# sony/DiffRoll

Hardware: AMD Instinct MI355X
Metric: piano-roll frames/sec (200-step sample) (higher is better)
Workload: dtype f32

## Files before the change

### diffroll_amd/build.py

```python
from __future__ import annotations

import os
import shutil
import subprocess
import sys

HERE = os.path.dirname(os.path.abspath(__file__))
CSRC = os.path.join(HERE, "csrc")
LIBDIR = os.path.join(HERE, "lib")
LIB = os.path.join(LIBDIR, "libdiffroll_amd.so")
SOURCES = ["gemm.hip", "stack.hip", "tail.hip", "update.hip", "threshold.hip", "rescale.hip", "project.hip", "momentum.hip", "frontend.hip", "pack.hip", "plan.hip", "abi.hip", "debug_abi.hip", "comm.hip"]
HEADERS = [os.path.join(CSRC, h) for h in ("kernels.h", "chain_tables.h", "device_common.h", "gemm_body.h", "persistent.h", "update_quad.h", "threshold_quad.h", "rescale_quad.h", "project_quad.h", "momentum_quad.h", "engine_state.h", "device_buffer.h", "captured_chain.h", "fused_mode.h", "launch_plan.h", "tenants.h")] + \
          [os.path.join(os.path.dirname(HERE), "include", h) for h in ("diffroll_amd.h", "diffroll_amd_debug.h")]
FLAGS = ["--offload-arch=gfx950", "-O3", "-std=c++17", "-fPIC", "-Wall", "-Wno-unused-function"]


def _hipcc() -> str:
    for cand in (os.environ.get("HIPCC"), shutil.which("hipcc"), "/opt/rocm/bin/hipcc"):
        if cand and os.path.exists(cand):
            return cand
    raise RuntimeError("hipcc not found (need ROCm with gfx950 support)")


def _stale(target: str, deps) -> bool:
    if not os.path.exists(target):
        return True
    t = os.path.getmtime(target)
    return any(os.path.getmtime(d) > t for d in deps)


VARIANTS = {
    "bounds": dict(flags=["-DDR_BOUNDS"], link=[]),
    "hook": dict(flags=["-DDR_FAULT_HOOK"], link=[]),
    "fault1": dict(flags=["-DDR_FAULT=1"], link=[]),
    "fault2": dict(flags=["-DDR_FAULT=2"], link=[]),
    "asan": dict(flags=["-O1", "-g", "-fsanitize=address,undefined", "-fno-gpu-sanitize", "-shared-libsan", "-fno-omit-frame-pointer"],
                 link=["-fsanitize=address,undefined", "-shared-libsan"]),
    "ubsan": dict(flags=["-O1", "-g", "-fsanitize=undefined", "-fno-sanitize-recover=undefined", "-fno-gpu-sanitize", "-fno-omit-frame-pointer"],
                  link=["-fsanitize=undefined", "-shared-libsan", "@RPATH:libclang_rt.ubsan_standalone-x86_64.so"]),
}


def variant_path(variant: str) -> str:
    return os.path.join(LIBDIR, f"libdiffroll_amd_{variant}.so")


def build(force: bool = False, verbose: bool = True, variant: str = "") -> str:
    hipcc = _hipcc()
    os.makedirs(LIBDIR, exist_ok=True)
    objdir = os.path.join(LIBDIR, "obj" + ("_" + variant if variant else ""))
    os.makedirs(objdir, exist_ok=True)
    extra = VARIANTS[variant] if variant else dict(flags=[], link=[])
    lib = variant_path(variant) if variant else LIB
    objs = []
    relink = force
    jobs = []
    wanted = {src.replace(".hip", ".o") for src in SOURCES}
    for name in os.listdir(objdir):
        if name not in wanted:
            os.remove(os.path.join(objdir, name))
            relink = True
    for src in SOURCES:
        s = os.path.join(CSRC, src)
        o = os.path.join(objdir, src.replace(".hip", ".o"))
        if force or _stale(o, [s] + HEADERS):
            jobs.append([hipcc] + FLAGS + extra["flags"] + ["-c", s, "-o", o])
        objs.append(o)
    if jobs:
        from concurrent.futures import ThreadPoolExecutor

        def run(cmd):
            if verbose:
                print(" ".join(cmd), flush=True)
            subprocess.check_call(cmd)
        with ThreadPoolExecutor(max_workers=min(len(jobs), os.cpu_count() or 4)) as ex:
            list(ex.map(run, jobs))
        relink = True
    if relink or _stale(lib, objs):
        link = []
        for f in extra["link"]:
            if f.startswith("@RPATH:"):
                rt = subprocess.check_output([hipcc, "-print-file-name=" + f[len("@RPATH:"):]], text=True).strip()
                link.append("-Wl,-rpath," + os.path.dirname(os.path.realpath(rt)))
            else:
                link.append(f)
        cmd = [hipcc, "--offload-arch=gfx950", "-shared", "-fPIC"] + link + objs + ["-ldl", "-o", lib]
        if verbose:
            print(" ".join(cmd), flush=True)
        subprocess.check_call(cmd)
    return lib


def asan_runtime() -> str:
    out = subprocess.check_output([_hipcc(), "-print-file-name=libclang_rt.asan-x86_64.so"], text=True).strip()
    return out


if __name__ == "__main__":
    var = ""
    for a in sys.argv[1:]:
        if a.startswith("--variant="):
            var = a.split("=", 1)[1]
    print(build(force="--force" in sys.argv, variant=var))
```

### diffroll_amd/csrc/gemm_body.h

```cpp
#pragma once
#include "device_common.h"

namespace dr {

DR_DEVINL void residual_quad(const float (&v)[4], const float4 bias, const float4 prev, float (&o)[4]) {
    float bb[4], pv[4];
    f4arr(bias, bb); f4arr(prev, pv);
#pragma unroll
    for (int e = 0; e < 4; ++e) o[e] = div_sqrt2(pv[e] + (v[e] + bb[e]));
}
DR_DEVINL void skip_quad(const float (&v)[4], const float4 bias, const float4 prev, const bool skip_init, float (&o)[4]) {
    float bb[4], pv[4];
    f4arr(bias, bb); f4arr(prev, pv);
#pragma unroll
    for (int e = 0; e < 4; ++e) o[e] = skip_init ? v[e] + bb[e] : (v[e] + bb[e]) + pv[e];
}
DR_DEVINL long cond_row(const GemmArgs& a, const int b) {
    int r = a.c_b0 + b;
    if (a.c_n > 0 && r >= a.c_n) r %= a.c_n;
    return r;
}
DR_DEVINL void gate_quad(const float (&v0)[4], const float (&v1)[4], const float4 bias0, const float4 bias1,
                         const float4 cond0, const float4 cond1, const bool has_c, float (&o)[4]) {
    float b0[4], b1[4], c0[4], c1[4];
    f4arr(bias0, b0); f4arr(bias1, b1);
    f4arr(cond0, c0); f4arr(cond1, c1);
#pragma unroll
    for (int e = 0; e < 4; ++e) {
        const float a0 = has_c ? b0[e] + c0[e] : b0[e];
        const float a1 = has_c ? b1[e] + c1[e] : b1[e];
        o[e] = gatef_(v0[e] + a0, v1[e] + a1);
    }
}
DR_DEVINL void hd_quad(const float (&h)[4], const float4 d, float (&o)[4]) {
    float dd[4];
    f4arr(d, dd);
#pragma unroll
    for (int e = 0; e < 4; ++e) o[e] = h[e] + dd[e];
}
template <int COH3, int COH4, int BF = 0>
DR_DEVINL void store_y2(const GemmArgs& a, const int b, const float (&o)[4], const float4 d, const int p0, const int t) {
    float o2[4];
    hd_quad(o, d, o2);
    if constexpr (BF) {
        store_bf16_quad<COH3>(a.Y2 + (long)b * a.y2_bs, o2, p0, t, a.T, a.wt_store);
    } else if (a.out_s3 & 2) {
        store_s3_quad<COH3>(a.Y2 + (long)b * a.y2_bs, o2, p0, t, a.T, a.y_rows >> 3, a.wt_store);
    } else {
        float* dst2 = a.Y2 + (long)b * a.y2_bs + (long)(p0 >> 2) * a.y_ps + (long)t * a.y_fs;
        store_f4<COH4>(dst2, make_float4(o2[0], o2[1], o2[2], o2[3]), a.wt_store);
    }
}

DR_DEVINL AF4 load_a4(const __amdgpu_buffer_rsrc_t wrsrc, const int wvo, const int slab, const int NS, const int code) {
    AF4 o;
#pragma unroll
    for (int g = 0; g < 4; ++g) {
        DR_CHECK(slab >= 0 && wvo + slab * 16384 + g * 4096 + 16 <= NS * 16384, code, slab, NS);
        o.v[g] = buffer_load_f4(wrsrc, wvo, slab * 16384 + g * 4096);
    }
    return o;
}

typedef __attribute__((address_space(3))) void* lds_ptr;

template <int BN, int AUX, class PlaneOf>
DR_DEVINL void dma_tile(float4* Rs, PlaneOf plane_of, const int T, const int t0, const int first, const int stride, const int lane, const int code) {
    constexpr int RWL = (BN + 63) / 64;
    for (int i = first; i < 32 * RWL; i += stride) {
        const int pl = i / RWL, seg = i - pl * RWL;
        const int f = seg * 64 + lane;
        const __amdgpu_buffer_rsrc_t rsrc = __builtin_amdgcn_make_buffer_rsrc((void*)plane_of(pl), 0, (unsigned)T * 16u, 0x00020000);
        if (BN % 64 == 0 || f < BN) {
            DR_CHECK_LDS(Rs + pl * BN + f, lds_off(Rs), lds_off(Rs) + 32u * BN * 16u, code);
            __builtin_amdgcn_raw_ptr_buffer_load_lds(rsrc, (lds_ptr)(Rs + pl * BN + seg * 64), 16, (t0 + f) * 16, 0, 0, AUX);
        }
    }
}

template <int KS, int PREC, int AUX, int RBN>
DR_DEVINL void producer(const GemmArgs& a, float4* Xs, float4* Rs, const int pw, const int lane, const int mt, const int b, const int t0,
                        const int halo, const int FW, const int c0, const int c1, const int code_x, const int code_r) {
    constexpr int XP = (PREC == 2 ? 4 : PREC ? 12 : 8) * KS;
    const int bx = a.x_bmod ? (b % a.x_bmod) : b;
    const float* Xg = a.X + (long)bx * a.x_bs;
    const int last_plane = a.x_planes - 1;
    const unsigned recs = ((unsigned)(a.T - 1) * (unsigned)a.x_fs + 4u) * 4u;
    const int wl = (FW + 63) >> 6;
    const int total = XP * wl;
    auto issue = [&](int chunk) {
        for (int i = pw; i < total; i += 4) {
            const int pl = i / wl, seg = i - pl * wl;
            const int f = seg * 64 + lane;
            const float* src;
            if constexpr (PREC == 2) {
                const int pc = min(chunk * (4 * KS) + pl, last_plane);
                src = Xg + (long)pc * a.x_ps;
            } else if constexpr (PREC) {
                const int sg = pl / 6, rem = pl - sg * 6, pce = rem >> 1, kq = rem & 1;
                const int pc = min(chunk * (4 * KS) + sg * 2 + kq, last_plane);
                src = Xg + (long)pce * a.x_piece + (long)pc * a.x_ps;
            } else {
                src = Xg + (long)min(chunk * XP + pl, last_plane) * a.x_ps;
            }
            const __amdgpu_buffer_rsrc_t rsrc = __builtin_amdgcn_make_buffer_rsrc((void*)src, 0, recs, 0x00020000);
            const int voff = (t0 - halo + f) * (int)a.x_fs * 4;
            float4* dst = Xs + (((chunk - c0) & 1) * XP + pl) * FW + seg * 64;
            if (f < FW) DR_CHECK_LDS(dst + lane, lds_off(Xs), lds_off(Xs) + 2u * XP * FW * 16u, code_x);
            if (f < FW) __builtin_amdgcn_raw_ptr_buffer_load_lds(rsrc, (lds_ptr)dst, 16, voff, 0, 0, AUX);
        }
    };
    if constexpr (RBN != 0) {
        auto plane_of = [&](int pl) -> const float* {
            const int row0 = mt * 128 + pl * 4;
            return (row0 < a.y_rows) ? a.Y + (long)b * a.y_bs + (long)(row0 >> 2) * a.y_ps
                                     : a.skip + (long)b * a.s_bs + (long)((row0 - a.y_rows) >> 2) * a.T * 4;
        };
        dma_tile<RBN, AUX>(Rs, plane_of, a.T, t0, pw, 4, lane, code_r);
    }
    issue(c0);
    for (int chunk = c0; chunk < c1; ++chunk) {
#if DR_FAULT != 1
        asm volatile("s_waitcnt vmcnt(0)" ::: "memory");
        __syncthreads();
#else
        __builtin_amdgcn_s_barrier();
#endif
        if (chunk + 1 < c1) issue(chunk + 1);
    }
}

template <int NI, int KS, int EPI, int PREC, int COH, int FOLDP = (NI == 1)>
DR_DEVINL void gemm_body(const GemmArgs& a, char* smem, const int mt, const int nt, const int ks) {
    constexpr int NW = (NI == 3 || NI == 5) ? NI : 2 * NI;
    constexpr int BN = 32 * NW;
    static_assert(NI == 1 || NI == 2 || ((NI == 3 || NI == 5) && EPI == EPI_GATE && PREC == 0 && KS == 1 && FOLDP == 1),
                  "block widths: 64, 128; 96, 160 (conv)");
    constexpr int XP = (PREC == 2 ? 4 : PREC ? 12 : 8) * KS;
    constexpr bool PAIRED = (EPI == EPI_GATE || EPI == EPI_POWER);
    int tid = threadIdx.x;
    if constexpr (COH) asm volatile("" : "+v"(tid));
    const int lane = tid & 63;
    const int wave = __builtin_amdgcn_readfirstlane(tid >> 6);
    const long long tick0 = a.dbg ? clock64() : 0;

    const int halo = ((a.taps - 1) >> 1) * a.dil;
    const int FW = BN + 2 * halo;
    float4* Xs = reinterpret_cast<float4*>(smem);
    float4* Rs = Xs + 2 * XP * FW;
#ifdef DR_BOUNDS
    const unsigned xs0 = lds_off(Xs), xs1 = xs0 + 2u * XP * FW * 16u, rs1 = xs1 + (EPI == EPI_RES_SKIP ? 32u * BN * 16u : 0u);
    if (tid == 0 && !COH) DR_CHECK(rs1 <= (unsigned)a.lds_bytes, 100, rs1, a.lds_bytes);
#endif

    const int tps = (a.T + BN - 1) / BN;
    const int b = nt / tps;
    const int t0 = (nt % tps) * BN;
    const int NS = a.kchunks * a.taps;
    const int cps = a.kchunks / KS / a.ksplit;
    const int c0 = ks * cps, c1 = c0 + cps;

    if (wave >= 4) {
        producer<KS, PREC, COH ? 16 : 0, EPI == EPI_RES_SKIP ? BN : 0>(a, Xs, Rs, wave - 4, lane, mt, b, t0, halo, FW, c0, c1, 101, 102);
        return;
    }

    const int r = lane & 31, hi = lane >> 5;

    f32x16 acc[NW];
#pragma unroll
    for (int ni = 0; ni < NW; ++ni)
#pragma unroll
        for (int e = 0; e < 16; ++e) acc[ni][e] = 0.f;
    f32x16 outer[NW];
#pragma unroll
    for (int ni = 0; ni < NW; ++ni)
#pragma unroll
        for (int e = 0; e < 16; ++e) outer[ni][e] = 0.f;
    const f32x16 zero16 = {0.f, 0.f, 0.f, 0.f, 0.f, 0.f, 0.f, 0.f, 0.f, 0.f, 0.f, 0.f, 0.f, 0.f, 0.f, 0.f};
    constexpr bool FOLD = FOLDP && EPI == EPI_GATE;
    auto fold = [&]() {
        if constexpr (FOLD) {
#pragma unroll
            for (int ni = 0; ni < NW; ++ni) outer[ni] = outer[ni] + acc[ni];
#pragma unroll
            for (int ni = 0; ni < NW; ++ni) asm volatile("" : "+v"(outer[ni]));
        }
    };

    float4 eop[NW][4];

    if constexpr (PREC == 2) {
        const __amdgpu_buffer_rsrc_t wrsrc = __builtin_amdgcn_make_buffer_rsrc(
            (void*)(a.Wp + (long)mt * NS * 2048), 0, (unsigned)NS * 8192u, 0x00020000);
        const int wvo = (hi * 128 + wave * 32 + r) * 16;
        auto load_ag = [&](int slab, int g) -> uint4 {
            DR_CHECK(slab >= 0 && wvo + slab * 8192 + g * 4096 + 16 <= NS * 8192, 113, slab, NS);
            return buffer_load_u4(wrsrc, wvo, slab * 8192 + g * 4096);
        };
        const int s0 = c0 * KS * a.taps;
        AF2 wA, wB;
        wA.v[0] = load_ag(s0, 0); wA.v[1] = load_ag(s0, 1);
        wB.v[0] = load_ag(min(s0 + 1, NS - 1), 0); wB.v[1] = load_ag(min(s0 + 1, NS - 1), 1);
        const int cen = (a.taps - 1) >> 1;
        const int per_chunk = a.taps * KS;
        const uint4* Xsb = reinterpret_cast<const uint4*>(Xs);
        struct BF1 { uint4 v[NW]; };
        BF1 b0, b1;
        auto xaddr = [&](int chunk, int q) -> const uint4* {
            const int j = q / KS, sub = q - j * KS;
            return Xsb + (((chunk - c0) & 1) * XP + sub * 4 + hi) * FW + halo + (j - cen) * a.dil + r;
        };
        auto rd1 = [&](const uint4* Xb, int g) -> BF1 {
            BF1 o;
#pragma unroll
            for (int ni = 0; ni < NW; ++ni) {
                DR_CHECK_LDS(Xb + g * 2 * FW + ni * 32, xs0, xs1, 114);
                o.v[ni] = Xb[g * 2 * FW + ni * 32];
            }
            return o;
        };
        auto mma1 = [&](auto FIRST, const uint4 af, const BF1& bf) {
            constexpr bool kFirst = FOLD && decltype(FIRST)::value;
#pragma unroll
            for (int ni = 0; ni < NW; ++ni) acc[ni] = mma_bf16(af, bf.v[ni], kFirst ? zero16 : acc[ni]);
        };
        auto step = [&](auto ROLE, auto FIRST, int slab, int chunk, int q) {
            constexpr bool kB = decltype(ROLE)::value;
            const uint4* Xb = xaddr(chunk, q);
            const int nx = min(slab + 2, NS - 1);
            b1 = rd1(Xb, 1);
            mma1(FIRST, kB ? wB.v[0] : wA.v[0], b0);
            if constexpr (kB) wB.v[0] = load_ag(nx, 0);
            else wA.v[0] = load_ag(nx, 0);
            b0 = rd1(xaddr(chunk, min(q + 1, per_chunk - 1)), 0);
            mma1(std::false_type{}, kB ? wB.v[1] : wA.v[1], b1);
            if constexpr (kB) wB.v[1] = load_ag(nx, 1);
            else wA.v[1] = load_ag(nx, 1);
            sgb<0x100, 1>();
            sgb_mix1<NW - 1, 0>(); sgb<0x8, 1>(); sgb<0x20, 1>();
            sgb<0x100, 1>();
            sgb_mix1<NW - 1, 0>(); sgb<0x8, 1>(); sgb<0x20, 1>();
        };
        using T_ = std::true_type;
        using F_ = std::false_type;
        for (int chunk = c0; chunk < c1; ++chunk) {
            auto at = [&](auto R, auto FIRST, int q) {
                const int j = q / KS, sub = q - j * KS;
                step(R, FIRST, (chunk * KS + sub) * a.taps + j, chunk, q);
            };
            __syncthreads();
            b0 = rd1(xaddr(chunk, 0), 0);
            fold();
            at(F_{}, T_{}, 0);
            int q = 1;
            for (; q + 2 <= per_chunk; q += 2) {
                at(T_{}, F_{}, q);
                at(F_{}, F_{}, q + 1);
            }
            if (q < per_chunk) at(T_{}, F_{}, q);
            else { const AF2 t = wA; wA = wB; wB = t; }
        }
    } else if constexpr (PREC == 1) {
        const __amdgpu_buffer_rsrc_t wrsrc = __builtin_amdgcn_make_buffer_rsrc(
            (void*)(a.Wp + (long)mt * NS * 6144), 0, (unsigned)NS * 24576u, 0x00020000);
        const int wvo = (hi * 128 + wave * 32 + r) * 16;
        auto load_a3 = [&](int slab) -> AF6 {
            AF6 o;
#pragma unroll
            for (int gp = 0; gp < 6; ++gp) {
                DR_CHECK(slab >= 0 && wvo + slab * 24576 + gp * 4096 + 16 <= NS * 24576, 103, slab, NS);
                o.v[gp] = buffer_load_u4(wrsrc, wvo, slab * 24576 + gp * 4096);
            }
            return o;
        };
        AF6 wA = load_a3(c0 * KS * a.taps), wB;
        const int cen = (a.taps - 1) >> 1;
        const int per_chunk = a.taps * KS;
        const uint4* Xs3 = reinterpret_cast<const uint4*>(Xs);
        struct BF3 { uint4 v[3][NW]; };
        BF3 b0, b1;
        auto xaddr = [&](int chunk, int q) -> const uint4* {
            const int j = q / KS, sub = q - j * KS;
            return Xs3 + (((chunk - c0) & 1) * XP + sub * 12 + hi) * FW + halo + (j - cen) * a.dil + r;
        };
        auto rd3 = [&](const uint4* Xb, int g) -> BF3 {
            BF3 o;
#pragma unroll
            for (int pz = 0; pz < 3; ++pz)
#pragma unroll
                for (int ni = 0; ni < NW; ++ni) {
                    DR_CHECK_LDS(Xb + (g * 6 + pz * 2) * FW + ni * 32, xs0, xs1, 104);
                    o.v[pz][ni] = Xb[(g * 6 + pz * 2) * FW + ni * 32];
                }
            return o;
        };
        auto mma6 = [&](auto FIRST, const uint4 a0, const uint4 a1, const uint4 a2, const BF3& bf) {
            constexpr bool kFirst = FOLD && decltype(FIRST)::value;
#pragma unroll
            for (int ni = 0; ni < NW; ++ni) acc[ni] = mma_bf16(a2, bf.v[0][ni], kFirst ? zero16 : acc[ni]);
#pragma unroll
            for (int ni = 0; ni < NW; ++ni) acc[ni] = mma_bf16(a0, bf.v[2][ni], acc[ni]);
#pragma unroll
            for (int ni = 0; ni < NW; ++ni) acc[ni] = mma_bf16(a1, bf.v[1][ni], acc[ni]);
// ... 361 lines not shown
#pragma unroll
    for (int ni = 0; ni < NW; ++ni)
#pragma unroll
        for (int e = 0; e < 16; ++e) acc[ni][e] = 0.f;

    AF4 aA = load_a(0), aB;
    BF bA = load_b(0), bB;
    auto step = [&](auto ROLE, int slab) {
        constexpr bool kB = decltype(ROLE)::value;
        const int nxt = min(slab + 1, NS - 1);
        if constexpr (kB) { aA = load_a(nxt); bA = load_b(nxt); }
        else { aB = load_a(nxt); bB = load_b(nxt); }
#pragma unroll
        for (int g = 0; g < 4; ++g) {
            const float4 af = kB ? aB.v[g] : aA.v[g];
#pragma unroll
            for (int ni = 0; ni < NW; ++ni) acc[ni] = __builtin_amdgcn_mfma_f32_32x32x2f32(af.x, (kB ? bB.v[g][ni] : bA.v[g][ni]).x, acc[ni], 0, 0, 0);
#pragma unroll
            for (int ni = 0; ni < NW; ++ni) acc[ni] = __builtin_amdgcn_mfma_f32_32x32x2f32(af.y, (kB ? bB.v[g][ni] : bA.v[g][ni]).y, acc[ni], 0, 0, 0);
#pragma unroll
            for (int ni = 0; ni < NW; ++ni) acc[ni] = __builtin_amdgcn_mfma_f32_32x32x2f32(af.z, (kB ? bB.v[g][ni] : bA.v[g][ni]).z, acc[ni], 0, 0, 0);
#pragma unroll
            for (int ni = 0; ni < NW; ++ni) acc[ni] = __builtin_amdgcn_mfma_f32_32x32x2f32(af.w, (kB ? bB.v[g][ni] : bA.v[g][ni]).w, acc[ni], 0, 0, 0);
        }
        constexpr int NLD = 4 + 4 * NW, PER = (16 * NW) / NLD;
        sgb_spread<NLD, PER>();
        sgb<0x8, 16 * NW - NLD * PER>();
    };
    const int rowb = mt * 128 + wave * 32 + 4 * hi;
    const bool res_rows = rowb < a.y_rows;
    float4 ebias[4], ed2[4], eop[RLDS ? 1 : NW][4];
    auto load_epilogue = [&]() {
#pragma unroll
        for (int q = 0; q < 4; ++q) {
            ebias[q] = *reinterpret_cast<const float4*>(a.bias + rowb + 8 * q);
            if constexpr (EPI == EPI_RES_SKIP)
                ed2[q] = *reinterpret_cast<const float4*>(a.d2 + (a.tsel ? (long)a.tsel[b] * a.d2_ts : 0) + min(rowb + 8 * q, a.y_rows - 4));
        }
        if constexpr (RLDS || EPI != EPI_RES_SKIP) return;
        const float* base = res_rows ? a.Y + (long)b * a.y_bs + (long)(rowb >> 2) * a.y_ps
                                     : a.skip + (long)b * a.s_bs + (long)((rowb - a.y_rows) >> 2) * a.T * 4;
        const long qs = res_rows ? 2 * a.y_ps : (long)2 * a.T * 4;
        const long fs = res_rows ? a.y_fs : 4;
#pragma unroll
        for (int ni = 0; ni < NW; ++ni) {
            const int tc = min(t0 + ni * 32 + r, a.T - 1);
#pragma unroll
            for (int q = 0; q < 4; ++q) eop[ni][q] = *reinterpret_cast<const float4*>(base + q * qs + tc * fs);
        }
    };
    int slab = 0;
    const int pre = max(NS - 2, 0) & ~1;
    for (; slab < pre; slab += 2) {
        step(std::false_type{}, slab);
        step(std::true_type{}, slab + 1);
        if (a.dbg && slab == 0 && blockIdx.x == 0 && threadIdx.x == 0) a.dbg[2] = clock64() - tick0;
    }
    if (a.dbg && blockIdx.x == 0 && threadIdx.x == 0) a.dbg[3] = clock64() - tick0;
    if constexpr (!RLDS) load_epilogue();
    __builtin_amdgcn_sched_barrier(0);
    for (; slab + 2 <= NS; slab += 2) {
        step(std::false_type{}, slab);
        step(std::true_type{}, slab + 1);
    }
    if (slab < NS) step(std::false_type{}, slab);
    const long long tick1 = a.dbg ? clock64() : 0;
    if constexpr (RLDS) load_epilogue();

#pragma unroll
    for (int ni = 0; ni < NW; ++ni) {
        const int t = t0 + ni * 32 + r;
        if (t >= a.T) continue;
#pragma unroll
        for (int q = 0; q < 4; ++q) {
            const int p0 = rowb + 8 * q;
            float v[4], o[4];
#pragma unroll
            for (int e = 0; e < 4; ++e) v[e] = acc[ni][4 * q + e];
            if constexpr (EPI != EPI_RES_SKIP) {
                if (p0 >= a.y_rows) continue;
                float bb[4];
                f4arr(ebias[q], bb);
#pragma unroll
                for (int e = 0; e < 4; ++e) {
                    o[e] = a.alpha * v[e] + bb[e];
                    if constexpr (EPI == EPI_RELU) o[e] = fmaxf(o[e], 0.f);
                }
                float* dst = a.Y + (long)b * a.y_bs + (long)(p0 >> 2) * a.y_ps + (long)t * a.y_fs;
                store_f4<COH>(dst, make_float4(o[0], o[1], o[2], o[3]), a.wt_store);
                continue;
            }
            float4* rs = nullptr;
            if constexpr (RLDS) rs = Rs + (wave * 8 + 2 * q + hi) * BN + foff + ni * 32 + r;
#ifdef DR_BOUNDS
            if constexpr (RLDS) DR_CHECK_LDS(rs, lds_off(Rs), lds_off(Rs) + 32u * BN * 16u, 121);
#endif
            float4 pv;
            if constexpr (RLDS) pv = *rs;
            else pv = eop[ni][q];
            if (res_rows) {
                float* dst = a.Y + (long)b * a.y_bs + (long)(p0 >> 2) * a.y_ps + (long)t * a.y_fs;
                residual_quad(v, ebias[q], pv, o);
                if constexpr (RLDS) *rs = make_float4(o[0], o[1], o[2], o[3]);
                else *reinterpret_cast<float4*>(dst) = make_float4(o[0], o[1], o[2], o[3]);
                if (a.Y2) store_y2<0, COH>(a, b, o, ed2[q], p0, t);
            } else {
                float* dst = a.skip + (long)b * a.s_bs + ((long)((p0 - a.y_rows) >> 2) * a.T + t) * 4;
                skip_quad(v, ebias[q], pv, a.skip_init, o);
                if constexpr (RLDS) *rs = make_float4(o[0], o[1], o[2], o[3]);
                else *reinterpret_cast<float4*>(dst) = make_float4(o[0], o[1], o[2], o[3]);
            }
        }
    }
    if (a.dbg && blockIdx.x == 0 && threadIdx.x == 0) {
        a.dbg[0] = tick1 - tick0;
        a.dbg[1] = clock64() - tick0;
    }
}

template <int NJ, int KS, int EPI>
DR_DEVINL void gemm16_body(const GemmArgs& a, char* smem, const int mt, const int nt) {
    static_assert(EPI == EPI_GATE || EPI == EPI_RES_SKIP, "16x16 variant: hot kernels only");
    constexpr int BN = 32 * NJ;
    constexpr int XP = 8 * KS;
    constexpr int RT = 2;
    constexpr int CT = 2 * NJ;

    const int tid = threadIdx.x;
    const int lane = tid & 63;
    const int wave = __builtin_amdgcn_readfirstlane(tid >> 6);
    const int halo = ((a.taps - 1) >> 1) * a.dil;
    const int FW = BN + 2 * halo;
    float4* Xs = reinterpret_cast<float4*>(smem);
    float4* Rs = Xs + 2 * XP * FW;
#ifdef DR_BOUNDS
    const unsigned xs0 = lds_off(Xs), xs1 = xs0 + 2u * XP * FW * 16u, rs1 = xs1 + (EPI == EPI_RES_SKIP ? 32u * BN * 16u : 0u);
    if (tid == 0) DR_CHECK(rs1 <= (unsigned)a.lds_bytes, 140, rs1, a.lds_bytes);
#endif

    const int tps = (a.T + BN - 1) / BN;
    const int b = nt / tps;
    const int t0 = (nt % tps) * BN;
    const int NS = a.kchunks * a.taps;
    const int nchunks = a.kchunks / KS;

    if (wave >= 4) {
        producer<KS, 0, 0, EPI == EPI_RES_SKIP ? BN : 0>(a, Xs, Rs, wave - 4, lane, mt, b, t0, halo, FW, 0, nchunks, 141, 142);
        return;
    }

    const int li = lane & 15, kq = lane >> 4;
    float4 acc[RT][CT];
#pragma unroll
    for (int rt = 0; rt < RT; ++rt)
#pragma unroll
        for (int ct = 0; ct < CT; ++ct) acc[rt][ct] = f4zero();

    const __amdgpu_buffer_rsrc_t wrsrc = __builtin_amdgcn_make_buffer_rsrc(
        (void*)(a.Wp + (long)mt * NS * 4096), 0, (unsigned)NS * 16384u, 0x00020000);
    const int wvo = (kq * 128 + wave * 32 + li) * 16;
    auto load_a = [&](int slab) -> AF4 {
        AF4 o;
#pragma unroll
        for (int g = 0; g < 2; ++g)
#pragma unroll
            for (int rt = 0; rt < RT; ++rt) {
                DR_CHECK(slab >= 0 && wvo + slab * 16384 + g * 8192 + rt * 256 + 16 <= NS * 16384, 143, slab, NS);
                o.v[g * RT + rt] = buffer_load_f4(wrsrc, wvo, slab * 16384 + g * 8192 + rt * 256);
            }
        return o;
    };
    AF4 wA = load_a(0), wB;
    const int cen = (a.taps - 1) >> 1;
    const int per_chunk = a.taps * KS;
    typedef float v4f __attribute__((ext_vector_type(4)));

    struct BF { float4 v[CT]; };
    BF b0, b1;
    auto xaddr = [&](int chunk, int q) -> const float4* {
        const int j = q / KS, sub = q - j * KS;
        return Xs + ((chunk & 1) * XP + sub * 8 + kq) * FW + halo + (j - cen) * a.dil + li;
    };
    auto rd = [&](const float4* Xb, int g) -> BF {
        BF o;
#pragma unroll
        for (int ct = 0; ct < CT; ++ct) {
            DR_CHECK_LDS(Xb + g * 4 * FW + ct * 16, xs0, xs1, 144);
            o.v[ct] = Xb[g * 4 * FW + ct * 16];
        }
        return o;
    };
    auto mma = [&](const float4 af, const BF& bf, int rt) {
#pragma unroll
        for (int ct = 0; ct < CT; ++ct) {
            v4f c = {acc[rt][ct].x, acc[rt][ct].y, acc[rt][ct].z, acc[rt][ct].w};
            c = __builtin_amdgcn_mfma_f32_16x16x4f32(af.x, bf.v[ct].x, c, 0, 0, 0);
            c = __builtin_amdgcn_mfma_f32_16x16x4f32(af.y, bf.v[ct].y, c, 0, 0, 0);
            c = __builtin_amdgcn_mfma_f32_16x16x4f32(af.z, bf.v[ct].z, c, 0, 0, 0);
            c = __builtin_amdgcn_mfma_f32_16x16x4f32(af.w, bf.v[ct].w, c, 0, 0, 0);
            acc[rt][ct] = make_float4(c[0], c[1], c[2], c[3]);
        }
    };
    auto step = [&](auto ROLE, int slab, int chunk, int q) {
        constexpr bool kB = decltype(ROLE)::value;
        const float4* Xb = xaddr(chunk, q);
        if constexpr (kB) wA = load_a(min(slab + 1, NS - 1));
        else wB = load_a(min(slab + 1, NS - 1));
        b1 = rd(Xb, 1);
#pragma unroll
        for (int rt = 0; rt < RT; ++rt) mma(kB ? wB.v[rt] : wA.v[rt], b0, rt);
        b0 = rd(xaddr(chunk, min(q + 1, per_chunk - 1)), 0);
#pragma unroll
        for (int rt = 0; rt < RT; ++rt) mma(kB ? wB.v[RT + rt] : wA.v[RT + rt], b1, rt);
        sgb<0x100, CT>(); sgb_spread<2 * RT, (4 * RT * CT) / (2 * RT)>();
        sgb<0x100, CT>(); sgb<0x8, 4 * RT * CT>();
    };
    using T_ = std::true_type;
    using F_ = std::false_type;
    for (int chunk = 0; chunk < nchunks; ++chunk) {
        auto at = [&](auto R, int q) {
            const int j = q / KS, sub = q - j * KS;
            step(R, (chunk * KS + sub) * a.taps + j, chunk, q);
        };
        __syncthreads();
        b0 = rd(xaddr(chunk, 0), 0);
        int q = 0;
        for (; q + 2 <= per_chunk; q += 2) {
            at(F_{}, q);
            at(T_{}, q + 1);
        }
        if (q < per_chunk) {
            at(F_{}, q);
            wA = wB;
        }
    }

    const int rowb = mt * 128 + wave * 32 + kq * 4;
    float4 ebias[RT], ed2[RT];
    const float* cbase = nullptr;
    if constexpr (EPI == EPI_GATE)
        cbase = (b < a.n_cond || !a.cond2) ? a.cond + (b < a.n_cond ? cond_row(a, b) : 0L) * a.c_bs : a.cond2;
    {
        const float* bsrc = a.bias;
        if constexpr (EPI == EPI_GATE) bsrc = (b < a.n_cond) ? a.bias : a.bias2;
#pragma unroll
        for (int rt = 0; rt < RT; ++rt) {
            ebias[rt] = *reinterpret_cast<const float4*>(bsrc + rowb + rt * 16);
            if constexpr (EPI == EPI_RES_SKIP)
                ed2[rt] = *reinterpret_cast<const float4*>(a.d2 + (a.tsel ? (long)a.tsel[b] * a.d2_ts : 0) + min(rowb + rt * 16, a.y_rows - 4));
        }
    }
#pragma unroll
    for (int ct = 0; ct < CT; ++ct) {
        const int t = t0 + ct * 16 + li;
        if constexpr (EPI == EPI_GATE) {
            float4 cnd[RT];
            const int tc = min(t, a.T - 1);
            const float* cb = cbase + (long)tc * 4;
#pragma unroll
            for (int rt = 0; rt < RT; ++rt) cnd[rt] = *reinterpret_cast<const float4*>(cb + (long)((rowb + rt * 16) >> 2) * a.T * 4);
            if (t >= a.T) continue;
            const bool has_c = b < a.n_cond || a.cond2 != nullptr;
            {
                const int c0 = mt * 64 + wave * 16 + kq * 4;
                if (c0 >= a.y_rows) continue;
                float v0[4], v1[4], o[4];
                f4arr(acc[0][ct], v0); f4arr(acc[1][ct], v1);
                gate_quad(v0, v1, ebias[0], ebias[1], cnd[0], cnd[1], has_c, o);
                if (a.out_s3 & 1) {
                    store_s3_quad(a.Y + (long)b * a.y_bs, o, c0, t, a.T, a.y_rows >> 3);
                } else {
                    float* dst = a.Y + (long)b * a.y_bs + (long)(c0 >> 2) * a.y_ps + (long)t * a.y_fs;
                    *reinterpret_cast<float4*>(dst) = make_float4(o[0], o[1], o[2], o[3]);
                }
            }
        } else {
            float4 pv4[RT];
#pragma unroll
            for (int rt = 0; rt < RT; ++rt) {
                DR_CHECK_LDS(Rs + ((wave * 32 + rt * 16) / 4 + kq) * BN + ct * 16 + li, xs1, rs1, 145);
                pv4[rt] = Rs[((wave * 32 + rt * 16) / 4 + kq) * BN + ct * 16 + li];
            }
            if (t >= a.T) continue;
#pragma unroll
            for (int rt = 0; rt < RT; ++rt) {
                const int p0 = rowb + rt * 16;
                float v[4], o[4];
                f4arr(acc[rt][ct], v);
                if (p0 < a.y_rows) {
                    float* dst = a.Y + (long)b * a.y_bs + (long)(p0 >> 2) * a.y_ps + (long)t * a.y_fs;
                    residual_quad(v, ebias[rt], pv4[rt], o);
                    *reinterpret_cast<float4*>(dst) = make_float4(o[0], o[1], o[2], o[3]);
                    if (a.Y2) store_y2<0, 0>(a, b, o, ed2[rt], p0, t);
                } else {
                    float* dst = a.skip + (long)b * a.s_bs + ((long)((p0 - a.y_rows) >> 2) * a.T + t) * 4;
                    skip_quad(v, ebias[rt], pv4[rt], a.skip_init, o);
                    *reinterpret_cast<float4*>(dst) = make_float4(o[0], o[1], o[2], o[3]);
                }
            }
        }
    }
}

}
```

### diffroll_amd/csrc/tail.hip

```cpp
#include "gemm_body.h"
#include "persistent.h"
#include "update_quad.h"

namespace dr {

DR_BOUNDS_TU(tail)

__global__ __launch_bounds__(512) void tail_kernel(const TailArgs s) {
    extern __shared__ __attribute__((aligned(16))) char smem[];
    float4* XT = reinterpret_cast<float4*>(smem);
    const int wave = __builtin_amdgcn_readfirstlane(threadIdx.x >> 6);
    const int lane = threadIdx.x & 63;
    const int MT = s.Cp >> 6;
    const int tps = (s.T + s.BN - 1) / s.BN;
    const unsigned gsize = (unsigned)(MT * tps);
    int grp, member;
    if (s.xcd_n) {
        const int xcd = blockIdx.x & 7, idx = blockIdx.x >> 3;
        member = idx % (int)gsize;
        grp = (idx / (int)gsize) * 8 + xcd;
    } else {
        member = blockIdx.x % (int)gsize;
        grp = blockIdx.x / (int)gsize;
    }
    if (grp >= s.NB) return;
    if (__hip_atomic_load(s.derr, __ATOMIC_RELAXED, __HIP_MEMORY_SCOPE_AGENT)) return;
    DR_CHECK(grp >= 0 && grp < 512, 150, grp, member);
    unsigned* ctr = s.bar + 4 * grp;
    const bool paired = s.dual > 0;
    const int pair_i = paired ? (grp < s.dual ? grp : grp - s.dual) : grp;
    const int pair_half = (paired && grp >= s.dual) ? 1 : 0;
    unsigned* pctr = s.pbar + 4 * pair_i;
    const int P = s.Cp >> 2;
    const long act_bs = (long)s.Cp * s.T;
    int mark_i = 0;
    auto mark = [&]() { if (s.dbg && blockIdx.x == 0 && threadIdx.x == 0) s.dbg[mark_i] = clock64(); ++mark_i; };
    mark();

    {
        GemmArgs a{};
        a.d2 = s.zero; a.wt_store = 1;
        a.Wp = s.skip_w; a.bias = s.skip_b; a.MT = (s.Cp + 127) >> 7; a.NB = s.NB; a.T = s.T; a.alpha = s.alpha;
        a.X = s.skip; a.x_bs = act_bs; a.x_ps = (long)s.T * 4; a.x_fs = 4; a.x_planes = P; a.kchunks = s.Cp >> 5;
        a.taps = 1; a.dil = 1; a.ksplit = 1;
        a.Y = s.tmp; a.y_bs = act_bs; a.y_ps = (long)s.T * 4; a.y_fs = 4; a.y_rows = s.Cp;
        const int tps64 = (s.T + 63) >> 6;
        const int n1 = a.MT * tps64;
        if (wave < 4)
            for (int it = member; it < n1; it += (int)gsize) pw_body<2, 1, 0, 64, EPI_RELU>(a, it % a.MT, grp * tps64 + it / a.MT, wave);
    }
    mark();
    group_barrier<true>(ctr, gsize + DR_FAULT_EXTRA(s), s.err, s.derr);
    mark();
    const int tps32 = (s.T + 31) >> 5;
    {
        GemmArgs a{};
        a.d2 = s.zero; a.wt_store = 1;
        a.Wp = s.outp_w; a.bias = s.outp_b; a.MT = 1; a.NB = s.NB; a.T = s.T; a.alpha = 1.f;
        a.X = s.tmp; a.x_bs = act_bs; a.x_ps = (long)s.T * 4; a.x_fs = 4; a.x_planes = P; a.kchunks = s.Cp >> 5;
        a.taps = 1; a.dil = 1; a.ksplit = 1;
        a.Y = s.x0; a.y_bs = (long)s.T * 88; a.y_ps = 4; a.y_fs = 88; a.y_rows = 88;
        if (wave < 3)
            for (int it = member; it < tps32; it += (int)gsize) pw_body<1, 1, 0, 32, EPI_PLAIN>(a, 0, grp * tps32 + it, wave);
    }
    mark();
    if (paired) group_barrier<true>(pctr, 2u * gsize + DR_FAULT_EXTRA(s), s.err, s.derr);
    else group_barrier<true>(ctr, 2u * (gsize + DR_FAULT_EXTRA(s)), s.err, s.derr);
    if (win_H(s.u) > 0) {
        if (threadIdx.x == 0) {
            const unsigned epoch = (s.u.dyn ? s.u.dyn->epoch : 0u) + s.epoch;
            if (member == 0 && pair_half == 0) __hip_atomic_store(s.ready + pair_i, epoch, __ATOMIC_RELAXED, __HIP_MEMORY_SCOPE_AGENT);
            const unsigned* tab = s.u.win_tab;
            const bool mine = pair_i < s.u_B;
            const bool lower = mine && (tab ? window_idx(tab[pair_i]) > 0 : pair_i > 0);
            const bool upper = mine && pair_i + 1 < s.u_B && (!tab || window_idx(tab[pair_i + 1]) > 0);
            neighbour_wait(s.ready, pair_i, lower, upper, epoch, s.err, s.derr);
        }
        __syncthreads();
    }
    mark();
    if (pair_i < s.u_B) {
        const int MTi = s.in_w ? ((s.Cp + 127) >> 7) : 1;
        const int n3 = MTi * tps32;
        const int stride = (int)gsize * (paired ? 2 : 1);
        const long roll0 = (long)pair_i * s.T * 88;
        for (int it = pair_half * (int)gsize + member; it < n3; it += stride) {
            const int mti = it % MTi, ck = it / MTi;
            const int f0 = ck * 32;
            __syncthreads();
            for (int q = threadIdx.x; q < 24 * 32; q += 512) {
                const int fi = q / 24, pl = q - fi * 24;
                float4 v = f4zero();
                if (pl < 22 && f0 + fi < s.T) {
                    const long i4 = (roll0 + (long)(f0 + fi) * 88 + pl * 4) >> 2;
                    float4 y;
                    v = update_quad(s.u, i4, &y);
                    if (mti == 0) {
                        reinterpret_cast<float4*>(s.x_out)[i4] = v;
                        if (s.u.mode == 5 && hist_next(s.u)) reinterpret_cast<float4*>(hist_next(s.u))[i4] = y;
                    }
                }
                DR_CHECK_LDS(XT + pl * 32 + fi, lds_off(XT), lds_off(XT) + 24u * 32u * 16u, 151);
                XT[pl * 32 + fi] = v;
            }
            if (!s.in_w) continue;
            __syncthreads();
            if (wave >= 4) continue;
            const int r = lane & 31, hi = lane >> 5;
            const __amdgpu_buffer_rsrc_t wr = __builtin_amdgcn_make_buffer_rsrc((void*)(s.in_w + (long)mti * 3 * 4096), 0, 3u * 16384u, 0x00020000);
            const int wvo = (hi * 128 + wave * 32 + r) * 16;
            f32x16 acc;
#pragma unroll
            for (int e = 0; e < 16; ++e) acc[e] = 0.f;
#pragma unroll
            for (int kc = 0; kc < 3; ++kc)
#pragma unroll
                for (int g = 0; g < 4; ++g) {
                    const float4 af = buffer_load_f4(wr, wvo, kc * 16384 + g * 4096);
                    DR_CHECK_LDS(XT + (kc * 8 + g * 2 + hi) * 32 + r, lds_off(XT), lds_off(XT) + 24u * 32u * 16u, 152);
                    const float4 bf = XT[(kc * 8 + g * 2 + hi) * 32 + r];
                    acc = __builtin_amdgcn_mfma_f32_32x32x2f32(af.x, bf.x, acc, 0, 0, 0);
                    acc = __builtin_amdgcn_mfma_f32_32x32x2f32(af.y, bf.y, acc, 0, 0, 0);
                    acc = __builtin_amdgcn_mfma_f32_32x32x2f32(af.z, bf.z, acc, 0, 0, 0);
                    acc = __builtin_amdgcn_mfma_f32_32x32x2f32(af.w, bf.w, acc, 0, 0, 0);
                }
            const int t = f0 + r;
            if (t >= s.T) continue;
#pragma unroll
            for (int q = 0; q < 4; ++q) {
                const int p0 = mti * 128 + wave * 32 + 8 * q + 4 * hi;
                if (p0 >= s.Cp) continue;
                const float4 bb = *reinterpret_cast<const float4*>(s.in_b + p0);
                const float4 dd = *reinterpret_cast<const float4*>(s.d2_next + p0);
                const float4 h4 = make_float4(fmaxf(acc[4 * q] + bb.x, 0.f), fmaxf(acc[4 * q + 1] + bb.y, 0.f),
                                              fmaxf(acc[4 * q + 2] + bb.z, 0.f), fmaxf(acc[4 * q + 3] + bb.w, 0.f));
                const float4 hd4 = make_float4(h4.x + dd.x, h4.y + dd.y, h4.z + dd.z, h4.w + dd.w);
                const long off = ((long)(p0 >> 2) * s.T + t) * 4;
                *reinterpret_cast<float4*>(s.h + (long)pair_i * act_bs + off) = h4;
                store_f4<1>(s.hd + (long)pair_i * act_bs + off, hd4, s.conv_w != nullptr);
                if (s.dual_next > 0) {
                    *reinterpret_cast<float4*>(s.h + (long)(pair_i + s.dual_next) * act_bs + off) = h4;
                    *reinterpret_cast<float4*>(s.hd + (long)(pair_i + s.dual_next) * act_bs + off) = hd4;
                }
            }
        }
    }
    mark();
    if (s.dual_next > 0 && s.conv_w) {
        if (paired) group_barrier<false>(pctr, 2u * (2u * gsize + DR_FAULT_EXTRA(s)), s.err, s.derr);
        else group_barrier<false>(ctr, 3u * (gsize + DR_FAULT_EXTRA(s)), s.err, s.derr);
        mark();
        GemmArgs a{};
        a.d2 = s.zero; a.wt_store = 0;
        a.lds_bytes = s.lds_bytes;
        a.MT = MT; a.NB = s.dual_next; a.T = s.T; a.alpha = 1.f; a.ksplit = 1;
        a.x_bs = act_bs; a.x_ps = (long)s.T * 4; a.x_fs = 4; a.x_planes = P; a.kchunks = s.Cp >> 5;
        a.y_bs = act_bs; a.y_ps = (long)s.T * 4; a.y_fs = 4; a.y_rows = s.Cp;
        a.Wp = s.conv_w; a.bias = s.conv_b; a.bias2 = s.conv_b2;
        a.X = s.hd; a.taps = s.taps; a.dil = s.dil;
        a.cond = s.cond; a.cond2 = s.cond2; a.c_bs = s.c_bs; a.c_n = s.c_n; a.n_cond = s.dual_next;
        a.dual = s.dual_next;
        a.Y = s.g;
        const int bn4 = s.t4_ni == 3 ? 96 : 64;
        const int tps4 = (s.T + bn4 - 1) / bn4;
        const int n4 = MT * tps4;
        for (int it = pair_half * (int)gsize + member; it < n4; it += (paired ? 2 : 1) * (int)gsize) {
            asm volatile("s_waitcnt vmcnt(0)" ::: "memory");
            __syncthreads();
            if (s.t4_ni == 3) gemm_body<3, 1, EPI_GATE, 0, 1, 1>(a, smem, it % MT, pair_i * tps4 + it / MT, 0);
            else if (s.fold) gemm_body<1, 1, EPI_GATE, 0, 1, 1>(a, smem, it % MT, pair_i * tps4 + it / MT, 0);
            else gemm_body<1, 1, EPI_GATE, 0, 1, 0>(a, smem, it % MT, pair_i * tps4 + it / MT, 0);
        }
    }
    if (s.dbg && blockIdx.x == 0 && threadIdx.x == 0) s.dbg[7] = clock64();
    if (threadIdx.x == 0) {
        const unsigned left = __hip_atomic_fetch_add(ctr + 1, 1u, __ATOMIC_RELAXED, __HIP_MEMORY_SCOPE_AGENT);
        if (left == gsize - 1) {
            __hip_atomic_store(ctr, 0u, __ATOMIC_RELAXED, __HIP_MEMORY_SCOPE_AGENT);
            __hip_atomic_store(ctr + 1, 0u, __ATOMIC_RELAXED, __HIP_MEMORY_SCOPE_AGENT);
        }
        if (paired) {
            const unsigned pleft = __hip_atomic_fetch_add(pctr + 1, 1u, __ATOMIC_RELAXED, __HIP_MEMORY_SCOPE_AGENT);
            if (pleft == 2u * gsize - 1u) {
                __hip_atomic_store(pctr, 0u, __ATOMIC_RELAXED, __HIP_MEMORY_SCOPE_AGENT);
                __hip_atomic_store(pctr + 1, 0u, __ATOMIC_RELAXED, __HIP_MEMORY_SCOPE_AGENT);
            }
        }
    }
}

hipError_t launch_tail(const TailArgs& s, hipStream_t st) {
    if (s.BN != 64 && s.BN != 128 && s.BN != 160) return hipErrorInvalidValue;
    if ((s.Cp & 63) || s.NB < 1 || s.T < 1) return hipErrorInvalidValue;
    if (s.dual > 0 && s.NB != 2 * s.dual) return hipErrorInvalidValue;
    if (s.dual_next < 0 || (s.dual_next > 0 && (s.dual_next != s.u_B || s.u_B != (s.dual > 0 ? s.dual : s.NB)))) return hipErrorInvalidValue;
    if (!s.x_out || s.x_out == s.u.x) return hipErrorInvalidValue;
    if (win_H(s.u) > 0 && (!s.ready || s.u_B > STACK_GROUPS || 2 * win_H(s.u) < s.T || win_H(s.u) >= s.T)) return hipErrorInvalidValue;
    if (s.u.win_tab && win_H(s.u) <= 0) return hipErrorInvalidValue;
    const int tps = (s.T + s.BN - 1) / s.BN, MT = s.Cp >> 6;
    TailArgs b = s;
    const int NBp = xcd_padded_groups(s.NB, MT * tps, &b.xcd_n);
    size_t lds = 24 * 32 * 16;
    if (s.conv_w) {
        if (s.dual_next <= 0 || !s.in_w || (s.taps & 1) == 0) return hipErrorInvalidValue;
        const long pair_blocks = (s.dual > 0 ? 2L : 1L) * MT * tps;
        const long n64 = (long)MT * ((s.T + 63) / 64), n96 = (long)MT * ((s.T + 95) / 96);
        const long c64 = (n64 + pair_blocks - 1) / pair_blocks * 64, c96 = (n96 + pair_blocks - 1) / pair_blocks * 96;
        b.t4_ni = (s.fold && s.t4_ni != 1 && (c96 < c64 || s.t4_ni == 3)) ? 3 : 1;
        lds = std::max(lds, gemm_lds_bytes(b.t4_ni, 1, s.taps, s.dil, 0, EPI_GATE));
        if (lds > 160 * 1024) return hipErrorInvalidValue;
    }
    b.lds_bytes = (int)lds;
    hipLaunchKernelGGL(tail_kernel, dim3((unsigned)(MT * tps * NBp)), dim3(512), lds, st, b);
    return hipGetLastError();
}

hipError_t init_tail_kernels() {
    return allow_max_lds(&tail_kernel);
}

}
```

Measured before the change: 2265.

## Fuse skip and output projections per 16-frame slab through LDS in tail kernel

```diff
diff --git a/diffroll_amd/build.py b/diffroll_amd/build.py
--- a/diffroll_amd/build.py
+++ b/diffroll_amd/build.py
@@ -10,7 +10,7 @@
 LIBDIR = os.path.join(HERE, "lib")
 LIB = os.path.join(LIBDIR, "libdiffroll_amd.so")
 SOURCES = ["gemm.hip", "stack.hip", "tail.hip", "update.hip", "threshold.hip", "rescale.hip", "project.hip", "momentum.hip", "frontend.hip", "pack.hip", "plan.hip", "abi.hip", "debug_abi.hip", "comm.hip"]
-HEADERS = [os.path.join(CSRC, h) for h in ("kernels.h", "chain_tables.h", "device_common.h", "gemm_body.h", "persistent.h", "update_quad.h", "threshold_quad.h", "rescale_quad.h", "project_quad.h", "momentum_quad.h", "engine_state.h", "device_buffer.h", "captured_chain.h", "fused_mode.h", "launch_plan.h", "tenants.h")] + \
+HEADERS = [os.path.join(CSRC, h) for h in ("kernels.h", "chain_tables.h", "device_common.h", "gemm_body.h", "slab_map.h", "persistent.h", "update_quad.h", "threshold_quad.h", "rescale_quad.h", "project_quad.h", "momentum_quad.h", "engine_state.h", "device_buffer.h", "captured_chain.h", "fused_mode.h", "launch_plan.h", "tenants.h")] + \
           [os.path.join(os.path.dirname(HERE), "include", h) for h in ("diffroll_amd.h", "diffroll_amd_debug.h")]
 FLAGS = ["--offload-arch=gfx950", "-O3", "-std=c++17", "-fPIC", "-Wall", "-Wno-unused-function"]
 
diff --git a/diffroll_amd/csrc/gemm_body.h b/diffroll_amd/csrc/gemm_body.h
--- a/diffroll_amd/csrc/gemm_body.h
+++ b/diffroll_amd/csrc/gemm_body.h
@@ -1,5 +1,6 @@
 #pragma once
 #include "device_common.h"
+#include "slab_map.h"
 
 namespace dr {
 
@@ -967,4 +968,150 @@
     }
 }
 
-}
+template <int EPI>
+DR_DEVINL void plain_quad(const float alpha, const float (&v)[4], const float4 bias, float (&o)[4]) {
+    float bb[4];
+    f4arr(bias, bb);
+#pragma unroll
+    for (int e = 0; e < 4; ++e) {
+        o[e] = alpha * v[e] + bb[e];
+        if constexpr (EPI == EPI_RELU) o[e] = fmaxf(o[e], 0.f);
+    }
+}
+DR_DEVINL float slab_pick(const float4 f, const int c) { return c == 0 ? f.x : c == 1 ? f.y : c == 2 ? f.z : f.w; }
+
+DR_DEVINL void slab_deal(const float4 f, float (&o)[2][2]) {
+    typedef unsigned u32x2 __attribute__((ext_vector_type(2)));
+    const u32x2 s0 = __builtin_amdgcn_permlane32_swap(__float_as_uint(f.x), __float_as_uint(f.y), false, false);
+    const u32x2 s1 = __builtin_amdgcn_permlane32_swap(__float_as_uint(f.z), __float_as_uint(f.w), false, false);
+    o[0][0] = __uint_as_float(s0[0]); o[1][0] = __uint_as_float(s0[1]);
+    o[0][1] = __uint_as_float(s1[0]); o[1][1] = __uint_as_float(s1[1]);
+}
+
+DR_DEVINL float4 slab_copy(const float4 f) {
+    float4 o;
+    asm volatile("v_mov_b32 %0, %4\n\tv_mov_b32 %1, %5\n\tv_mov_b32 %2, %6\n\tv_mov_b32 %3, %7"
+                 : "=&v"(o.x), "=&v"(o.y), "=&v"(o.z), "=&v"(o.w) : "v"(f.x), "v"(f.y), "v"(f.z), "v"(f.w));
+    return o;
+}
+
+template <int NT>
+DR_DEVINL void slab_skip_body(const GemmArgs& a, const int b, const int t0, const int rt0, float4* ST) {
+    static_assert(NT == 1 || NT == 2 || NT == 4, "row tiles per wave");
+    int lane = threadIdx.x & 63;
+    asm volatile("" : "+v"(lane));
+    const int NS = a.kchunks;
+    const __amdgpu_buffer_rsrc_t wr = __builtin_amdgcn_make_buffer_rsrc(
+        (void*)(a.Wp + (long)(rt0 >> 3) * NS * 4096), 0, (unsigned)NS * 16384u, 0x00020000);
+    const __amdgpu_buffer_rsrc_t xr = __builtin_amdgcn_make_buffer_rsrc(
+        (void*)(a.X + (long)b * a.x_bs), 0, (unsigned)(a.x_planes * a.x_ps * 4), 0x00020000);
+    const int xps = (int)a.x_ps * 4;
+    const int wvo = slab16_a_pair_offset(lane, rt0 & 7);
+    const int xvo = slab16_b_pair_plane(lane) * xps + min(t0 + (lane & 15), a.T - 1) * 16;
+
+    struct FR { float4 a[2][NT], b[2]; };
+    auto load = [&](int slab) -> FR {
+        FR o;
+#pragma unroll
+        for (int gp = 0; gp < 2; ++gp) {
+#pragma unroll
+            for (int i = 0; i < NT; ++i) {
+                DR_CHECK(slab >= 0 && wvo + slab * 16384 + gp * 8192 + i * 256 + 16 <= NS * 16384, 153, slab, NS);
+                o.a[gp][i] = buffer_load_f4(wr, wvo, slab * 16384 + gp * 8192 + i * 256);
+            }
+            o.b[gp] = buffer_load_f4(xr, xvo, (slab * 8 + gp * 4) * xps);
+        }
+        return o;
+    };
+    f32x4 acc[NT];
+#pragma unroll
+    for (int i = 0; i < NT; ++i) acc[i] = f32x4{0.f, 0.f, 0.f, 0.f};
+    FR fA = load(0), fB;
+    auto step = [&](auto ROLE, int slab) {
+        constexpr bool kB = decltype(ROLE)::value;
+        const int nxt = min(slab + 1, NS - 1);
+        if constexpr (kB) fA = load(nxt);
+        else fB = load(nxt);
+        __builtin_amdgcn_sched_barrier(0);
+#pragma unroll
+        for (int gp = 0; gp < 2; ++gp) {
+            float bo[2][2], ao[NT][2][2];
+            float4 fb = slab_copy(kB ? fB.b[gp] : fA.b[gp]), fa[NT];
+#pragma unroll
+            for (int i = 0; i < NT; ++i) fa[i] = slab_copy(kB ? fB.a[gp][i] : fA.a[gp][i]);
+            slab_deal(fb, bo);
+#pragma unroll
+            for (int i = 0; i < NT; ++i) slab_deal(fa[i], ao[i]);
+#pragma unroll
+            for (int q = 0; q < 2; ++q)
+#pragma unroll
+                for (int j = 0; j < 2; ++j)
+#pragma unroll
+                    for (int i = 0; i < NT; ++i) acc[i] = __builtin_amdgcn_mfma_f32_16x16x4f32(ao[i][q][j], bo[q][j], acc[i], 0, 0, 0);
+        }
+        __builtin_amdgcn_sched_barrier(0);
+    };
+    int slab = 0;
+    for (; slab + 2 <= NS; slab += 2) {
+        step(std::false_type{}, slab);
+        step(std::true_type{}, slab + 1);
+    }
+    if (slab < NS) step(std::false_type{}, slab);
+#pragma unroll
+    for (int i = 0; i < NT; ++i) {
+        const int p0 = (rt0 + i) * 16 + 4 * ((lane >> 4) & 3);
+        const float v[4] = {acc[i][0], acc[i][1], acc[i][2], acc[i][3]};
+        float o[4];
+        plain_quad<EPI_RELU>(a.alpha, v, *reinterpret_cast<const float4*>(a.bias + p0), o);
+        float4* dst = ST + slab16_d_index(lane, rt0 + i);
+        DR_CHECK_LDS(dst, lds_off(ST), lds_off(ST) + (unsigned)a.x_planes * (SLAB_FRAMES * 16u), 154);
+        *dst = make_float4(o[0], o[1], o[2], o[3]);
+    }
+}
+
+DR_DEVINL void slab_out_body(const GemmArgs& a, const int b, const int t0, const int rt, const float4* ST) {
+    int lane = threadIdx.x & 63;
+    asm volatile("" : "+v"(lane));
+    const int NS = a.kchunks;
+    const __amdgpu_buffer_rsrc_t wr = __builtin_amdgcn_make_buffer_rsrc((void*)a.Wp, 0, (unsigned)NS * 16384u, 0x00020000);
+    const int wvo = slab16_a_offset(lane, rt);
+    const int c0 = slab16_component(lane, 0), c1 = slab16_component(lane, 1);
+    auto load_a = [&](int slab) { return load_a4(wr, wvo, slab, NS, 155); };
+    f32x4 acc = {0.f, 0.f, 0.f, 0.f};
+    AF4 wA = load_a(0), wB;
+    auto step = [&](auto ROLE, int slab) {
+        constexpr bool kB = decltype(ROLE)::value;
+        if constexpr (kB) wA = load_a(min(slab + 1, NS - 1));
+        else wB = load_a(min(slab + 1, NS - 1));
+        float4 bf[4];
+#pragma unroll
+        for (int g = 0; g < 4; ++g) {
+            const float4* src = ST + slab16_b_index(lane, slab, g);
+            DR_CHECK_LDS(src, lds_off(ST), lds_off(ST) + (unsigned)a.x_planes * (SLAB_FRAMES * 16u), 156);
+            bf[g] = *src;
+        }
+        __builtin_amdgcn_sched_barrier(0);
+#pragma unroll
+        for (int g = 0; g < 4; ++g) {
+            const float4 af = kB ? wB.v[g] : wA.v[g];
+            acc = __builtin_amdgcn_mfma_f32_16x16x4f32(slab_pick(af, c0), slab_pick(bf[g], c0), acc, 0, 0, 0);
+            acc = __builtin_amdgcn_mfma_f32_16x16x4f32(slab_pick(af, c1), slab_pick(bf[g], c1), acc, 0, 0, 0);
+        }
+        __builtin_amdgcn_sched_barrier(0);
+    };
+    int slab = 0;
+    for (; slab + 2 <= NS; slab += 2) {
+        step(std::false_type{}, slab);
+        step(std::true_type{}, slab + 1);
+    }
+    if (slab < NS) step(std::false_type{}, slab);
+    const int p0 = rt * 16 + 4 * (lane >> 4), t = t0 + (lane & 15);
+    if (p0 >= a.y_rows || t >= a.T) return;
+    const float v[4] = {acc[0], acc[1], acc[2], acc[3]};
+    float o[4];
+    plain_quad<EPI_PLAIN>(a.alpha, v, *reinterpret_cast<const float4*>(a.bias + p0), o);
+    float* dst = a.Y + (long)b * a.y_bs + (long)(p0 >> 2) * a.y_ps + (long)t * a.y_fs;
+    store_f4<1>(dst, make_float4(o[0], o[1], o[2], o[3]), a.wt_store);
+}
+
+}
diff --git a/diffroll_amd/csrc/slab_map.h b/diffroll_amd/csrc/slab_map.h
--- /dev/null
+++ b/diffroll_amd/csrc/slab_map.h
@@ -0,0 +1,31 @@
+#pragma once
+
+#if defined(__HIPCC__) || defined(__CUDACC__)
+#define DR_HD __host__ __device__ __forceinline__
+#else
+#define DR_HD inline
+#endif
+
+namespace dr {
+
+constexpr int SLAB_FRAMES = 16;
+
+DR_HD constexpr int slab_count(const int T) { return (T + SLAB_FRAMES - 1) / SLAB_FRAMES; }
+DR_HD constexpr int slab_of(const int member, const int round, const int gsize) { return member + round * gsize; }
+
+DR_HD constexpr int mfma32_channel(const int g, const int e, const int lane) { return 8 * g + 4 * (lane >> 5) + e; }
+DR_HD constexpr int mfma32_position(const int g, const int e, const int lane) { return (4 * g + e) * 2 + (lane >> 5); }
+
+DR_HD constexpr int slab16_half(const int lane) { return (lane >> 4) & 1; }
+DR_HD constexpr int slab16_component(const int lane, const int j) { return 2 * j + ((lane >> 5) & 1); }
+DR_HD constexpr int slab16_channel(const int g, const int j, const int lane) { return 8 * g + 4 * slab16_half(lane) + slab16_component(lane, j); }
+DR_HD constexpr int slab16_position(const int g, const int j, const int lane) { return (2 * g + j) * 4 + ((lane >> 4) & 3); }
+
+DR_HD constexpr int slab16_a_offset(const int lane, const int tile) { return (slab16_half(lane) * 128 + tile * 16 + (lane & 15)) * 16; }
+DR_HD constexpr int slab16_pair_group(const int lane, const int gp) { return 2 * gp + ((lane >> 5) & 1); }
+DR_HD constexpr int slab16_a_pair_offset(const int lane, const int tile) { return ((lane >> 5) & 1) * 4096 + slab16_a_offset(lane, tile); }
+DR_HD constexpr int slab16_b_pair_plane(const int lane) { return ((lane >> 5) & 1) * 2 + slab16_half(lane); }
+DR_HD constexpr int slab16_b_index(const int lane, const int step, const int g) { return (step * 8 + g * 2 + slab16_half(lane)) * SLAB_FRAMES + (lane & 15); }
+DR_HD constexpr int slab16_d_index(const int lane, const int rt) { return (rt * 4 + ((lane >> 4) & 3)) * SLAB_FRAMES + (lane & 15); }
+
+}
diff --git a/diffroll_amd/csrc/tail.hip b/diffroll_amd/csrc/tail.hip
--- a/diffroll_amd/csrc/tail.hip
+++ b/diffroll_amd/csrc/tail.hip
@@ -33,39 +33,37 @@
     unsigned* pctr = s.pbar + 4 * pair_i;
     const int P = s.Cp >> 2;
     const long act_bs = (long)s.Cp * s.T;
-    int mark_i = 0;
-    auto mark = [&]() { if (s.dbg && blockIdx.x == 0 && threadIdx.x == 0) s.dbg[mark_i] = clock64(); ++mark_i; };
-    mark();
+    auto mark = [&](const int i) { if (s.dbg && blockIdx.x == 0 && threadIdx.x == 0) s.dbg[i] = clock64(); };
+    mark(0);
 
     {
-        GemmArgs a{};
-        a.d2 = s.zero; a.wt_store = 1;
-        a.Wp = s.skip_w; a.bias = s.skip_b; a.MT = (s.Cp + 127) >> 7; a.NB = s.NB; a.T = s.T; a.alpha = s.alpha;
-        a.X = s.skip; a.x_bs = act_bs; a.x_ps = (long)s.T * 4; a.x_fs = 4; a.x_planes = P; a.kchunks = s.Cp >> 5;
-        a.taps = 1; a.dil = 1; a.ksplit = 1;
-        a.Y = s.tmp; a.y_bs = act_bs; a.y_ps = (long)s.T * 4; a.y_fs = 4; a.y_rows = s.Cp;
-        const int tps64 = (s.T + 63) >> 6;
-        const int n1 = a.MT * tps64;
-        if (wave < 4)
-            for (int it = member; it < n1; it += (int)gsize) pw_body<2, 1, 0, 64, EPI_RELU>(a, it % a.MT, grp * tps64 + it / a.MT, wave);
-    }
-    mark();
-    group_barrier<true>(ctr, gsize + DR_FAULT_EXTRA(s), s.err, s.derr);
-    mark();
+        float4* ST = reinterpret_cast<float4*>(smem);
+        GemmArgs a1{};
+        a1.Wp = s.skip_w; a1.bias = s.skip_b; a1.T = s.T; a1.alpha = s.alpha; a1.kchunks = s.Cp >> 5;
+        a1.X = s.skip; a1.x_bs = act_bs; a1.x_ps = (long)s.T * 4; a1.x_fs = 4; a1.x_planes = P;
+        GemmArgs a2{};
+        a2.Wp = s.outp_w; a2.bias = s.outp_b; a2.T = s.T; a2.alpha = 1.f; a2.kchunks = s.Cp >> 5; a2.x_planes = P;
+        a2.Y = s.x0; a2.y_bs = (long)s.T * 88; a2.y_ps = 4; a2.y_fs = 88; a2.y_rows = 88; a2.wt_store = 1;
+        const int RT = s.Cp >> 4;
+        const int nslab = slab_count(s.T);
+        for (int rd = 0; slab_of(member, rd, (int)gsize) < nslab; ++rd) {
+            const int t0 = slab_of(member, rd, (int)gsize) * SLAB_FRAMES;
+            if (rd) __syncthreads();
+            if ((RT & 31) == 0) {
+                for (int rt = wave * 4; rt < RT; rt += 32) slab_skip_body<4>(a1, grp, t0, rt, ST);
+            } else {
+                for (int rt = wave; rt < RT; rt += 8) slab_skip_body<1>(a1, grp, t0, rt, ST);
+            }
+            mark(1);
+            __syncthreads();
+            mark(2);
+            if (wave < 6) slab_out_body(a2, grp, t0, wave, ST);
+            mark(3);
+        }
+    }
     const int tps32 = (s.T + 31) >> 5;
-    {
-        GemmArgs a{};
-        a.d2 = s.zero; a.wt_store = 1;
-        a.Wp = s.outp_w; a.bias = s.outp_b; a.MT = 1; a.NB = s.NB; a.T = s.T; a.alpha = 1.f;
-        a.X = s.tmp; a.x_bs = act_bs; a.x_ps = (long)s.T * 4; a.x_fs = 4; a.x_planes = P; a.kchunks = s.Cp >> 5;
-        a.taps = 1; a.dil = 1; a.ksplit = 1;
-        a.Y = s.x0; a.y_bs = (long)s.T * 88; a.y_ps = 4; a.y_fs = 88; a.y_rows = 88;
-        if (wave < 3)
-            for (int it = member; it < tps32; it += (int)gsize) pw_body<1, 1, 0, 32, EPI_PLAIN>(a, 0, grp * tps32 + it, wave);
-    }
-    mark();
     if (paired) group_barrier<true>(pctr, 2u * gsize + DR_FAULT_EXTRA(s), s.err, s.derr);
-    else group_barrier<true>(ctr, 2u * (gsize + DR_FAULT_EXTRA(s)), s.err, s.derr);
+    else group_barrier<true>(ctr, gsize + DR_FAULT_EXTRA(s), s.err, s.derr);
     if (win_H(s.u) > 0) {
         if (threadIdx.x == 0) {
             const unsigned epoch = (s.u.dyn ? s.u.dyn->epoch : 0u) + s.epoch;
@@ -78,7 +76,7 @@
         }
         __syncthreads();
     }
-    mark();
+    mark(4);
     if (pair_i < s.u_B) {
         const int MTi = s.in_w ? ((s.Cp + 127) >> 7) : 1;
         const int n3 = MTi * tps32;
@@ -145,11 +143,11 @@
             }
         }
     }
-    mark();
+    mark(5);
     if (s.dual_next > 0 && s.conv_w) {
         if (paired) group_barrier<false>(pctr, 2u * (2u * gsize + DR_FAULT_EXTRA(s)), s.err, s.derr);
-        else group_barrier<false>(ctr, 3u * (gsize + DR_FAULT_EXTRA(s)), s.err, s.derr);
-        mark();
+        else group_barrier<false>(ctr, 2u * (gsize + DR_FAULT_EXTRA(s)), s.err, s.derr);
+        mark(6);
         GemmArgs a{};
         a.d2 = s.zero; a.wt_store = 0;
         a.lds_bytes = s.lds_bytes;
@@ -200,7 +198,8 @@
     const int tps = (s.T + s.BN - 1) / s.BN, MT = s.Cp >> 6;
     TailArgs b = s;
     const int NBp = xcd_padded_groups(s.NB, MT * tps, &b.xcd_n);
-    size_t lds = 24 * 32 * 16;
+    size_t lds = std::max<size_t>(24 * 32 * 16, (size_t)s.Cp * (SLAB_FRAMES * 4));
+    if (lds > 160 * 1024) return hipErrorInvalidValue;
     if (s.conv_w) {
         if (s.dual_next <= 0 || !s.in_w || (s.taps & 1) == 0) return hipErrorInvalidValue;
         const long pair_blocks = (s.dual > 0 ? 2L : 1L) * MT * tps;
```

Result: no change. 2263 (-0.1%).
